# vbronetskyi/nclt-slam-project

Measured on AMD Instinct MI355X. Metric: relocalization frames/sec @640x480, 10k-landmark DB; Hamming-match HBM GB/s, higher is better.
Workload: dtype u8; 1 GPU; 640x480 BGR frames, 10000-record landmark DB (640000 descriptors, rows=fixed64), global relocalization tick per frame: ORB(500) + whole-DB mutual Hamming scan + top-25 PnP-RANSAC(200); frames resident in HBM, every frame's 96-byte result record written to pinned host memory by the tick's last kernel; distinct_frames=32, preroll_steps=20, streams=4, records=10000, descriptors=640000, parallelism=frames sharded across ranks, database replicated, no collective

## Files before the change

nclt-slam-project_amd/csrc/reloc_orb.hip:

```cpp
#include <math.h>

#include "../../include/reloc_orb_pattern.h"
#include "reloc_internal.h"
#include "reloc_pixels.h"

static_assert(HARRIS_CHUNK == 1024, "k_harris reads one dword per thread");

__constant__ signed char c_pattern[RELOC_ORB_NTESTS * 4];
__constant__ int c_umax[16] = {15, 15, 15, 15, 14, 14, 14, 13, 13, 12, 11, 10, 9, 8, 6, 3};
__constant__ signed char c_ring_dx[16] = {0, 1, 2, 3, 3, 3, 2, 1, 0, -1, -2, -3, -3, -3, -2, -1};
__constant__ signed char c_ring_dy[16] = {3, 3, 2, 1, 0, -1, -2, -3, -3, -3, -2, -1, 0, 1, 2, 3};

__device__ __forceinline__ int find_level(const int *base, int id)
{
    int l = 0;
#pragma unroll
    for (int k = 1; k < NLEV; ++k) l += id >= base[k];
    return l;
}


struct OrbBatch { OrbFrame f[RELOC_BATCH_MAX]; };

__device__ __forceinline__ void pyr_tab_index(const OrbTable *__restrict__ tab, const PyrTile &T, const int (&tbase)[NLEV + 1], int i,
                                              int &po, int &pc)
{
    int j = i, nw = 0, x0 = 0, y0 = 0, ox = 0, cx = 0, oy = 0, cy = 0;
#pragma unroll
    for (int k = 1; k < NLEV; ++k) {
        const bool m = i >= tbase[k];
        j = m ? i - tbase[k] : j;
        nw = m ? T.n[k][1] - T.n[k][0] : nw;
        x0 = m ? (int)T.n[k][0] : x0;
        y0 = m ? (int)T.n[k][2] : y0;
        ox = m ? tab->rz_off[k][0] : ox;
        cx = m ? tab->rz_off[k][1] : cx;
        oy = m ? tab->rz_off[k][2] : oy;
        cy = m ? tab->rz_off[k][3] : cy;
    }
    const bool isx = j < nw;
    const int p = isx ? x0 + j : y0 + j - nw;
    po = (isx ? ox : oy) + p;
    pc = (isx ? cx : cy) + p;
}

__device__ __forceinline__ int pyr_div(int q, float inv) { return (int)(((float)q + 0.5f) * inv); }

template <int CH, bool ALIGNED, int PYR_BS>
__device__ __forceinline__ void pyramid_body(const OrbTable *__restrict__ tab, const PyrTile *__restrict__ tiles,
                                                 const int32_t *__restrict__ rz, const uint8_t *__restrict__ src, int w, int h,
                                                 int sstride, int order_rgb, uint8_t *__restrict__ pyr, PyrLds lds,
                                                 int32_t *__restrict__ hist, int32_t *__restrict__ cand_cnt)
{
    extern __shared__ u32 s_pyr[];
    const int tid = threadIdx.x;
    if (blockIdx.x == 0) {
        for (int i = tid; i < NLEV * 256; i += PYR_BS) hist[i] = 0;
        if (tid < NLEV) cand_cnt[tid] = 0;
    }
    const PyrTile &T = tiles[blockIdx.x];
    uint8_t *const base = reinterpret_cast<uint8_t *>(s_pyr);
    u32 *const tabs = s_pyr + (lds.tabs >> 2);
    int tbase[NLEV + 1];
    tbase[1] = 0;
#pragma unroll
    for (int l = 1; l < NLEV; ++l) tbase[l + 1] = tbase[l] + (T.n[l][1] - T.n[l][0]) + (T.n[l][3] - T.n[l][2]);
    constexpr int TAB_IT = 1024 / PYR_BS, L0_IT = 1536 / PYR_BS;
    u32 tv[TAB_IT][2];
#pragma unroll
    for (int it = 0; it < TAB_IT; ++it) {
        const int i = tid + it * PYR_BS;
        tv[it][0] = tv[it][1] = 0;
        if (i < tbase[NLEV]) {
            int po, pc;
            pyr_tab_index(tab, T, tbase, i, po, pc);
            tv[it][0] = (u32)rz[po];
            tv[it][1] = (u32)rz[pc];
        }
    }
    const int x00 = T.n[0][0], y00 = T.n[0][2], qpr0 = (T.n[0][1] - x00 + 3) >> 2, nq0 = qpr0 * (T.n[0][3] - y00);
    const float inv0 = 1.0f / (float)(qpr0 > 0 ? qpr0 : 1);
    u32 fv[L0_IT][3];
#pragma unroll
    for (int it = 0; it < L0_IT; ++it) {
        const int q = tid + it * PYR_BS;
        if (q < nq0) {
            const int ry = pyr_div(q, inv0), x4 = x00 + (q - ry * qpr0) * 4;
            pyr_fetch<CH, ALIGNED>(src + (size_t)(y00 + ry) * sstride + CH * x4, x4, w, fv[it]);
        }
    }
#pragma unroll
    for (int it = 0; it < TAB_IT; ++it) {
        const int i = tid + it * PYR_BS;
        if (i < tbase[NLEV]) tabs[i] = tv[it][0] | tv[it][1] << 16;
    }
#pragma unroll
    for (int it = 0; it < L0_IT; ++it) {
        const int q = tid + it * PYR_BS;
        if (q < nq0) {
            const int ry = pyr_div(q, inv0), x4 = x00 + (q - ry * qpr0) * 4;
            reinterpret_cast<u32 *>(base + lds.lev[0])[q] = pyr_gray4<CH>(fv[it], x4, w, order_rgb);
        }
    }
    for (int q = tid + L0_IT * PYR_BS; q < nq0; q += PYR_BS) {
        const int ry = pyr_div(q, inv0), x4 = x00 + (q - ry * qpr0) * 4;
        u32 d[3];
        pyr_fetch<CH, ALIGNED>(src + (size_t)(y00 + ry) * sstride + CH * x4, x4, w, d);
        reinterpret_cast<u32 *>(base + lds.lev[0])[q] = pyr_gray4<CH>(d, x4, w, order_rgb);
    }
    for (int i = tid + TAB_IT * PYR_BS; i < tbase[NLEV]; i += PYR_BS) {
        int po, pc;
        pyr_tab_index(tab, T, tbase, i, po, pc);
        tabs[i] = (u32)rz[po] | (u32)rz[pc] << 16;
    }
    __syncthreads();
#pragma unroll
    for (int l = 0; l + 1 < NLEV; ++l) {
        const int sw = tab->lev[l].w, sh = tab->lev[l].h;
        const uint8_t *cur = base + lds.lev[l];
        u32 *nxt = reinterpret_cast<u32 *>(base + lds.lev[l + 1]);
        const int nx0 = T.n[l][0], ny0 = T.n[l][2], pitch = ((T.n[l][1] - nx0 + 3) >> 2) << 2;
        const int dx0 = T.n[l + 1][0], dx1 = T.n[l + 1][1], dh = T.n[l + 1][3] - T.n[l + 1][2];
        const int qpr = (dx1 - dx0 + 3) >> 2;
        const u32 *xt = tabs + tbase[l + 1], *yt = xt + (dx1 - dx0);
        const u32 one = 1u << RELOC_RESIZE_COEF_BITS;
        const float inv = 1.0f / (float)(qpr > 0 ? qpr : 1);
        for (int q = tid; q < qpr * dh; q += PYR_BS) {
            const int ry = pyr_div(q, inv), rx4 = (q - ry * qpr) * 4;
            const u32 ye = yt[ry];
            const int sy0 = (int)(ye & 0xFFFF), sy1 = sy0 + 1 < sh ? sy0 + 1 : sh - 1;
            const u32 b = ye >> 16;
            const uint8_t *r0 = cur + (sy0 - ny0) * pitch - nx0, *r1 = cur + (sy1 - ny0) * pitch - nx0;
            u32 out = 0;
#pragma unroll
            for (int k = 0; k < 4; ++k) {
                if (dx0 + rx4 + k < dx1) {
                    const u32 xe = xt[rx4 + k];
                    const int k0 = (int)(xe & 0xFFFF), k1 = k0 + 1 < sw ? k0 + 1 : sw - 1;
                    const u32 a = xe >> 16;
                    const u32 h0 = (u32)r0[k0] * (one - a) + (u32)r0[k1] * a;
                    const u32 h1 = (u32)r1[k0] * (one - a) + (u32)r1[k1] * a;
                    const u32 v = h0 * (one - b) + h1 * b;
                    out |= ((v + (1u << 15)) >> 16) << (8 * k);
                }
            }
            nxt[q] = out;
        }
        __syncthreads();
    }
#pragma unroll
    for (int l = 0; l < NLEV; ++l) {
        const OrbLevel L = tab->lev[l];
        const uint8_t *cur = base + lds.lev[l];
        const int nx0 = T.n[l][0], ny0 = T.n[l][2], pitch = ((T.n[l][1] - nx0 + 3) >> 2) << 2;
        const int x0 = T.o[l][0], x1 = T.o[l][1], y0 = T.o[l][2], oh = T.o[l][3] - y0;
        const int qpr = (x1 - x0) >> 2;
        uint8_t *dst = pyr + L.off;
        const float inv = 1.0f / (float)(qpr > 0 ? qpr : 1);
        for (int q = tid; q < qpr * oh; q += PYR_BS) {
            const int ry = pyr_div(q, inv), x4 = x0 + (q - ry * qpr) * 4;
            u32 v = 0;
            if (x4 < L.w) {
                v = *reinterpret_cast<const u32 *>(cur + (y0 + ry - ny0) * pitch + (x4 - nx0));
                if (x4 + 4 > L.w) v &= 0xFFFFFFFFu >> (8 * (x4 + 4 - L.w));
            }
            *reinterpret_cast<u32 *>(dst + (size_t)(y0 + ry) * L.stride + x4) = v;
        }
    }
}
template <int CH, bool ALIGNED, int PYR_BS>
__global__ __launch_bounds__(PYR_BS) void k_pyramid(const OrbTable *__restrict__ tab, const PyrTile *__restrict__ tiles,
                                                 const int32_t *__restrict__ rz, const uint8_t *__restrict__ src, int w, int h,
                                                 int sstride, int order_rgb, uint8_t *__restrict__ pyr, PyrLds lds,
                                                 int32_t *__restrict__ hist, int32_t *__restrict__ cand_cnt)
{
    RELOC_SMALL_KERNEL_PRIO();
    pyramid_body<CH, ALIGNED, PYR_BS>(tab, tiles, rz, src, w, h, sstride, order_rgb, pyr, lds, hist, cand_cnt);
}
template <int CH, bool ALIGNED, int PYR_BS>
__global__ __launch_bounds__(PYR_BS) void k_pyramid_batch(OrbBatch b, int w, int h, int sstride, int order_rgb, PyrLds lds)
{
    RELOC_SMALL_KERNEL_PRIO();
    const OrbFrame &F = b.f[blockIdx.y];
    pyramid_body<CH, ALIGNED, PYR_BS>(F.tab, F.tiles, F.rz, F.src, w, h, sstride, order_rgb, F.pyr, lds, F.hist, F.cand_cnt);
}

template <bool REFLECT>
__device__ __forceinline__ u32 halo_dword(const uint8_t *__restrict__ row, int gx, int w)
{
    if (gx >= 0 && gx + 4 <= w) return *reinterpret_cast<const u32 *>(row + gx);
    u32 v = 0;
#pragma unroll
    for (int k = 0; k < 4; ++k) {
        const int x = REFLECT ? reflect101(gx + k, w) : min(max(gx + k, 0), w - 1);
        v |= (u32)row[x] << (8 * k);
    }
    return v;
}

constexpr int BT_P = BT_W / 4 + 2;
static_assert(BT_W == 64 && BT_H == 16, "blur7_tile maps 256 lanes to 16 rows x 16 dwords");
__device__ __forceinline__ void blur7_tile(const OrbTable *__restrict__ tab, const uint8_t *__restrict__ pyr,
                                           uint8_t *__restrict__ blur, int bid)
{
    __shared__ u32 s_in[(BT_H + 6) * BT_P];
    __shared__ u32 s_h[(BT_H + 6) * BT_W / 2];
    const int l = find_level(tab->blur_tile_base, bid);
    const OrbLevel L = tab->lev[l];
    const int tile = bid - tab->blur_tile_base[l];
    const int tx = (L.w + BT_W - 1) / BT_W;
    const int x0 = (tile % tx) * BT_W, y0 = (tile / tx) * BT_H;
    const uint8_t *src = pyr + L.off;
    const int tid = threadIdx.x;
    const int r16 = tid >> 4, c16 = tid & 15;
    {
        const int e = tid - 6 * 16;
        const bool edge = e >= 0;
        const int rb = edge ? e >> 1 : BT_H + r16, db = edge ? (e & 1) * (BT_P - 1) : 1 + c16;
        const bool on = e < 2 * (BT_H + 6);
        const int gya = reflect101(y0 + r16 - 3, L.h), gyb = reflect101(y0 + rb - 3, L.h);
        const u32 va = halo_dword<true>(src + (size_t)gya * L.stride, x0 + 4 * c16, L.w);
        u32 vb = 0;
        if (on) vb = halo_dword<true>(src + (size_t)gyb * L.stride, x0 - 4 + 4 * db, L.w);
        s_in[r16 * BT_P + 1 + c16] = va;
        if (on) s_in[rb * BT_P + db] = vb;
    }
    __syncthreads();
    constexpr u32 W_LO = RELOC_BLUR_K0 | RELOC_BLUR_K1 << 8 | RELOC_BLUR_K2 << 16 | (u32)RELOC_BLUR_K3 << 24;
    constexpr u32 W_HI = RELOC_BLUR_K2 | RELOC_BLUR_K1 << 8 | RELOC_BLUR_K0 << 16;
    static_assert(RELOC_BLUR_K3 < 256 && 2 * (RELOC_BLUR_K0 + RELOC_BLUR_K1 + RELOC_BLUR_K2) + RELOC_BLUR_K3 <= 256, "blur taps");
#pragma unroll
    for (int t = 0; t < 2; ++t) {
        const int ry = t * BT_H + r16;
        if (ry < BT_H + 6) {
            const u32 *p = s_in + ry * BT_P + c16;
            const u32 d0 = p[0], d1 = p[1], d2 = p[2];
            u32 s[4];
#pragma unroll
            for (int k = 0; k < 4; ++k) {
                const u32 lo = k < 3 ? __builtin_amdgcn_alignbyte(d1, d0, 1 + k) : d1;
                const u32 hi = k < 3 ? __builtin_amdgcn_alignbyte(d2, d1, 1 + k) : d2;
                s[k] = __builtin_amdgcn_udot4(lo, W_LO, __builtin_amdgcn_udot4(hi, W_HI, 0u, false), false);
            }
            *reinterpret_cast<uint2 *>(s_h + ry * (BT_W / 2) + 2 * c16) = make_uint2(s[0] | s[1] << 16, s[2] | s[3] << 16);
        }
    }
    __syncthreads();
    {
        u32 c[7][4];
#pragma unroll
        for (int j = 0; j < 7; ++j) {
            const uint2 d = *reinterpret_cast<const uint2 *>(s_h + (r16 + j) * (BT_W / 2) + 2 * c16);
            c[j][0] = d.x & 0xFFFF; c[j][1] = d.x >> 16; c[j][2] = d.y & 0xFFFF; c[j][3] = d.y >> 16;
        }
        u32 out = 0;
#pragma unroll
        for (int k = 0; k < 4; ++k) {
            const u32 s = RELOC_BLUR_K0 * (c[0][k] + c[6][k]) + RELOC_BLUR_K1 * (c[1][k] + c[5][k]) +
                          RELOC_BLUR_K2 * (c[2][k] + c[4][k]) + RELOC_BLUR_K3 * c[3][k];
            out |= ((s + (1u << 15)) >> 16) << (8 * k);
        }
        const int gy = y0 + r16, gx = x0 + 4 * c16;
        if (gy < L.h && gx < L.stride) *reinterpret_cast<u32 *>(blur + L.off + (size_t)gy * L.stride + gx) = out;
    }
}

__device__ int fast_is_corner(const uint8_t *p, int stride, int thr)
{
    const int c = p[0];
    u32 bright = 0, dark = 0;
#pragma unroll
    for (int k = 0; k < 16; ++k) {
        const int v = (int)p[c_ring_dy[k] * stride + c_ring_dx[k]] - c;
        bright |= (u32)(v > thr) << k;
        dark |= (u32)(v < -thr) << k;
    }
    auto run9 = [](u32 m) {
        u32 x = m | (m << 16);
        u32 y = x & (x >> 1);
        y &= y >> 2;
        y &= y >> 4;
        y &= x >> 8;
        return (y & 0xFFFFu) != 0;
    };
    return run9(bright) ? 1 : (run9(dark) ? -1 : 0);
}

__device__ int fast_corner_score(const uint8_t *p, int stride, int thr, int sign)
{
    const int c = p[0];
    int v[16];
#pragma unroll
    for (int k = 0; k < 16; ++k) v[k] = sign * ((int)p[c_ring_dy[k] * stride + c_ring_dx[k]] - c);
    int m2[16], m4[16], best = 0;
#pragma unroll
    for (int k = 0; k < 16; ++k) m2[k] = min(v[k], v[(k + 1) & 15]);
#pragma unroll
    for (int k = 0; k < 16; ++k) m4[k] = min(m2[k], m2[(k + 2) & 15]);
#pragma unroll
    for (int k = 0; k < 16; ++k) {
        const int m8 = min(m4[k], m4[(k + 4) & 15]);
        const int m9 = min(m8, v[(k + 8) & 15]);
        best = max(best, m9);
    }
    return best > thr ? best - 1 : 0;
}

__device__ __forceinline__ bool fast_run9(u32 x)
{
    u32 y = x & (x >> 1);
    y &= y >> 2;
    y &= y >> 4;
    y &= x >> 8;
    return (y & 0xFFFFu) != 0;
}

struct FastQuad {
    u32 nb[2], nd[2];
    const u32 (*w)[3];
    __device__ __forceinline__ FastQuad(const u32 (&rows)[7][3], int thr) : w(rows)
    {
        const u32 c = rows[3][1];
        const u32 ce = c & 0x00FF00FFu, co = (c >> 8) & 0x00FF00FFu;
        const u32 t2 = (0x7FFFu - (u32)thr) * 0x00010001u;
        nb[0] = t2 - ce; nb[1] = t2 - co;
        nd[0] = t2 + ce; nd[1] = t2 + co;
    }
    template <int DX, int DY>
    __device__ __forceinline__ void flags(u32 (&tb)[2], u32 (&td)[2]) const
    {
        constexpr int b = 4 + DX, q = b >> 2, o = b & 3;
        constexpr u32 sel_e = (u32)o | 0x0C00u | (u32)(o + 2) << 16 | 0x0C000000u;
        constexpr u32 sel_o = (u32)(o + 1) | 0x0C00u | (u32)(o + 3) << 16 | 0x0C000000u;
        const u32 ve = __builtin_amdgcn_perm(w[DY + 3][q + 1], w[DY + 3][q], sel_e);
        const u32 vo = __builtin_amdgcn_perm(w[DY + 3][q + 1], w[DY + 3][q], sel_o);
        tb[0] = ve + nb[0]; tb[1] = vo + nb[1];
        td[0] = nd[0] - ve; td[1] = nd[1] - vo;
    }
    template <int K>
    __device__ __forceinline__ void ring(u32 (&tb)[2], u32 (&td)[2]) const
    {
        constexpr int dx[16] = {0, 1, 2, 3, 3, 3, 2, 1, 0, -1, -2, -3, -3, -3, -2, -1};
        constexpr int dy[16] = {3, 3, 2, 1, 0, -1, -2, -3, -3, -3, -2, -1, 0, 1, 2, 3};
        flags<dx[K], dy[K]>(tb, td);
    }
    __device__ __forceinline__ bool candidate() const
    {
        u32 b0[2], d0[2], b4[2], d4[2], b8[2], d8[2], b12[2], d12[2];
        ring<0>(b0, d0); ring<4>(b4, d4); ring<8>(b8, d8); ring<12>(b12, d12);
        u32 any = 0;
#pragma unroll
        for (int j = 0; j < 2; ++j) {
            any |= (b0[j] & b4[j]) | (b8[j] & b12[j]) | ((b0[j] | b4[j]) & (b8[j] | b12[j]));
            any |= (d0[j] & d4[j]) | (d8[j] & d12[j]) | ((d0[j] | d4[j]) & (d8[j] | d12[j]));
        }
        return (any & 0x80008000u) != 0;
    }
    template <int K>
    __device__ __forceinline__ void shift_in(u32 (&mb)[2], u32 (&md)[2]) const
    {
        u32 tb[2], td[2];
        ring<K>(tb, td);
#pragma unroll
        for (int j = 0; j < 2; ++j) {
            mb[j] = (tb[j] & 0x80008000u) | ((mb[j] >> 1) & 0x7FFF7FFFu);
            md[j] = (td[j] & 0x80008000u) | ((md[j] >> 1) & 0x7FFF7FFFu);
        }
        if constexpr (K < 15) shift_in<K + 1>(mb, md);
    }
    __device__ __forceinline__ void masks(u32 (&mb)[2], u32 (&md)[2]) const
    {
        mb[0] = mb[1] = md[0] = md[1] = 0;
        shift_in<0>(mb, md);
    }
};

constexpr int FT_P = FT / 4 + 3;
static_assert(FT == 32, "fast_nms_tile maps 256 lanes to 32 rows x 8 dwords");
template <bool MASKED, int THR>
__device__ __forceinline__ void fast_nms_tile(const OrbTable *__restrict__ tab, const uint8_t *__restrict__ pyr,
                                              uint8_t *__restrict__ nms, int32_t *__restrict__ hist, int bid,
                                              const uint8_t *__restrict__ mask)
{
    __shared__ u32 s_img4[(FT + 8) * FT_P];
    __shared__ u32 s_sc4[(FT + 2) * (FT + 4) / 4];
    __shared__ unsigned short s_corner[(FT + 2) * (FT + 2)];
    __shared__ int s_nc;
    __shared__ int s_hist[256];
    const uint8_t *const s_img = reinterpret_cast<const uint8_t *>(s_img4);
    uint8_t *const s_sc = reinterpret_cast<uint8_t *>(s_sc4);
    const int l = find_level(tab->fast_tile_base, bid);
    const OrbLevel L = tab->lev[l];
    const int tile = bid - tab->fast_tile_base[l];
    const int tx = L.stride / FT;
    const int x0 = (tile % tx) * FT, y0 = (tile / tx) * FT;
    const int tid = threadIdx.x;
    const int e = RELOC_ORB_EDGE;
    const int thr = THR ? THR : tab->fast_thr;
    uint8_t *out = nms + L.off;
    const bool live = L.quota > 0 && x0 + FT > e && x0 < L.w - e && y0 + FT > e && y0 < L.h - e;
    if (!live) {
        const int y = y0 + tid / 8, x = x0 + (tid % 8) * 4;
        if (y < L.h) *reinterpret_cast<u32 *>(out + (size_t)y * L.stride + x) = 0;
        return;
    }
    s_hist[tid] = 0;
    const uint8_t *src = pyr + L.off;
    const int IS = 4 * FT_P;
    {
        const int r16 = tid >> 4, c16 = tid & 15;
        u32 v[3];
#pragma unroll
        for (int t = 0; t < 3; ++t) {
            const int ry = 16 * t + r16;
            if (c16 < FT / 4 + 2 && ry < FT + 8) {
                const int gy = min(max(y0 + ry - 4, 0), L.h - 1);
                v[t] = halo_dword<false>(src + (size_t)gy * L.stride, x0 - 4 + 4 * c16, L.w);
            }
        }
#pragma unroll
        for (int t = 0; t < 3; ++t) {
            const int ry = 16 * t + r16;
            if (c16 < FT / 4 + 2 && ry < FT + 8) s_img4[ry * FT_P + c16] = v[t];
        }
    }
    for (int i = tid; i < (FT + 2) * (FT + 4) / 4; i += 256) s_sc4[i] = 0;
    if (tid == 0) s_nc = 0;
    __syncthreads();
    const int SS = FT + 4;
    {
        const int ry = 1 + (tid >> 3), g = tid & 7, rx = 1 + 4 * g;
        u32 w[7][3];
#pragma unroll
        for (int r = 0; r < 7; ++r)
#pragma unroll
            for (int q = 0; q < 3; ++q) w[r][q] = s_img4[(ry + r) * FT_P + g + q];
        const FastQuad Q(w, thr);
        if (__any(Q.candidate())) {
            u32 mb[2], md[2];
            Q.masks(mb, md);
            const int gy = y0 + ry - 1;
            const bool row_in = gy >= 3 && gy < L.h - 3;
#pragma unroll
            for (int k = 0; k < 4; ++k) {
                const u32 sel = (k & 2) ? 0x03020302u : 0x01000100u;
                const bool br = fast_run9(__builtin_amdgcn_perm(mb[k & 1], mb[k & 1], sel));
                const bool dk = fast_run9(__builtin_amdgcn_perm(md[k & 1], md[k & 1], sel));
                const int gx = x0 + rx - 1 + k;
                if ((br || dk) && row_in && gx >= 3 && gx < L.w - 3)
                    s_corner[atomicAdd(&s_nc, 1)] = (unsigned short)((ry << 6) | (rx + k) | (br ? 0 : 0x8000));
            }
        }
    }
    {
        const int i = tid;
        const int ry = i < FT + 2 ? 0 : (i < 2 * (FT + 2) ? FT + 1 : (i < 3 * FT + 4 ? i - (2 * FT + 3) : i - (3 * FT + 3)));
        const int rx = i < FT + 2 ? i : (i < 2 * (FT + 2) ? i - (FT + 2) : (i < 3 * FT + 4 ? 0 : FT + 1));
        const int gy = y0 + ry - 1, gx = x0 + rx - 1;
        int pol = 0;
        bool cand = false;
        const uint8_t *pc = s_img + (ry + 3) * IS + (rx + 3);
        const bool inside = i < 4 * FT + 4 && gx >= 3 && gx < L.w - 3 && gy >= 3 && gy < L.h - 3;
        if (inside) {
            const int c = pc[0];
            const int v0 = (int)pc[3 * IS] - c, v4 = (int)pc[3] - c, v8 = (int)pc[-3 * IS] - c, v12 = (int)pc[-3] - c;
            const int nb = (v0 > thr) + (v4 > thr) + (v8 > thr) + (v12 > thr);
            const int nd = (v0 < -thr) + (v4 < -thr) + (v8 < -thr) + (v12 < -thr);
            cand = nb >= 2 || nd >= 2;
        }
// ... 807 lines not shown
```

nclt-slam-project_amd/csrc/reloc_pixels.h:

```cpp
#pragma once
#include "reloc_internal.h"

typedef uint32_t u32;

__device__ __forceinline__ int reflect101(int p, int n)
{
    if (n == 1) return 0;
    while (p < 0 || p >= n) {
        if (p < 0) p = -p;
        if (p >= n) p = 2 * n - 2 - p;
    }
    return p;
}

__device__ __forceinline__ int gray_fixed(int b, int g, int r, int flags)
{
    const bool c15 = flags & RELOC_GRAY_FLAG_15BIT;
    const int cb = c15 ? RELOC_GRAY15_CB : RELOC_GRAY_CB, cg = c15 ? RELOC_GRAY15_CG : RELOC_GRAY_CG, cr = c15 ? RELOC_GRAY15_CR : RELOC_GRAY_CR;
    const int sh = c15 ? RELOC_GRAY15_SHIFT : RELOC_GRAY_SHIFT;
    return (b * cb + g * cg + r * cr + (1 << (sh - 1))) >> sh;
}
static inline int gray_flags(const reloc_ctx *ctx, int order)
{
    return (order & 1) | (ctx->prm.gray_coeff_bits == RELOC_GRAY15_SHIFT ? RELOC_GRAY_FLAG_15BIT : 0);
}

template <int CH, bool ALIGNED>
__device__ __forceinline__ void pyr_fetch(const uint8_t *sp, int x4, int w, u32 (&d)[3])
{
    if (ALIGNED) {
        const u32 *s4 = reinterpret_cast<const u32 *>(sp);
        d[0] = s4[0];
        if (CH == 3) { d[1] = s4[1]; d[2] = s4[2]; }
    } else {
        d[0] = d[1] = d[2] = 0;
#pragma unroll
        for (int k = 0; k < 4 * CH; ++k)
            if (x4 + k / CH < w) d[k >> 2] |= (u32)sp[k] << (8 * (k & 3));
    }
}

template <int CH>
__device__ __forceinline__ u32 pyr_gray4(const u32 (&d)[3], int x4, int w, int order_rgb)
{
    if (CH == 1) return d[0];
    u32 out = 0;
#pragma unroll
    for (int k = 0; k < 4; ++k) {
        int c[3];
#pragma unroll
        for (int j = 0; j < 3; ++j) { const int bi = 3 * k + j; c[j] = (d[bi >> 2] >> (8 * (bi & 3))) & 0xFF; }
        const int b = (order_rgb & 1) ? c[2] : c[0], r = (order_rgb & 1) ? c[0] : c[2];
        const int g = gray_fixed(b, c[1], r, order_rgb);
        if (x4 + k < w) out |= (u32)g << (8 * k);
    }
    return out;
}
```

Baseline: 7648 frames/s.

## Restructure pyramid kernel walks into column-major row strides with scalar tile loads

Replaces the per-element float division index decomposition in the pyramid build with a precomputed per-thread column/row walk, using a constant reciprocal table. Tile rectangles and the table are read through the constant address space so they load as scalars. The per-level resize hoists the x coefficients out of the row loop, packs output with a byte permute and masks the tail instead of branching. Gray conversion drops the per-pixel channel-swap select and the width check on aligned frames. These changes cut VALU and address arithmetic in a small ORB stage, at the cost of more intricate indexing and reliance on undocumented layout asserts.

```diff
diff --git a/nclt-slam-project_amd/csrc/reloc_orb.hip b/nclt-slam-project_amd/csrc/reloc_orb.hip
--- a/nclt-slam-project_amd/csrc/reloc_orb.hip
+++ b/nclt-slam-project_amd/csrc/reloc_orb.hip
@@ -22,29 +22,61 @@
 
 struct OrbBatch { OrbFrame f[RELOC_BATCH_MAX]; };
 
-__device__ __forceinline__ void pyr_tab_index(const OrbTable *__restrict__ tab, const PyrTile &T, const int (&tbase)[NLEV + 1], int i,
-                                              int &po, int &pc)
-{
-    int j = i, nw = 0, x0 = 0, y0 = 0, ox = 0, cx = 0, oy = 0, cy = 0;
-#pragma unroll
-    for (int k = 1; k < NLEV; ++k) {
-        const bool m = i >= tbase[k];
-        j = m ? i - tbase[k] : j;
-        nw = m ? T.n[k][1] - T.n[k][0] : nw;
-        x0 = m ? (int)T.n[k][0] : x0;
-        y0 = m ? (int)T.n[k][2] : y0;
-        ox = m ? tab->rz_off[k][0] : ox;
-        cx = m ? tab->rz_off[k][1] : cx;
-        oy = m ? tab->rz_off[k][2] : oy;
-        cy = m ? tab->rz_off[k][3] : cy;
-    }
+#define PYR_CONST __attribute__((address_space(4)))
+typedef const PYR_CONST OrbTable *PyrTabP;
+template <class P>
+__device__ __forceinline__ P pyr_reload(P p)
+{
+    asm volatile("" : "+s"(p));
+    return p;
+}
+struct PyrRect { int x0, x1, y0, y1; };
+__device__ __forceinline__ PyrRect pyr_rect(const PYR_CONST u32 *tile, int r)
+{
+    const u32 a = tile[2 * r], b = tile[2 * r + 1];
+    return {(int)(a & 0xFFFF), (int)(a >> 16), (int)(b & 0xFFFF), (int)(b >> 16)};
+}
+static_assert(offsetof(PyrTile, n) == 8 * NLEV && sizeof(PyrTile) == 16 * NLEV, "pyr_rect reads a rectangle as two dwords");
+
+__device__ __forceinline__ void pyr_tab_index(PyrTabP tab, const PyrRect &N, int l, int j, int &po, int &pc)
+{
+    const int nw = N.x1 - N.x0;
     const bool isx = j < nw;
-    const int p = isx ? x0 + j : y0 + j - nw;
-    po = (isx ? ox : oy) + p;
-    pc = (isx ? cx : cy) + p;
-}
-
-__device__ __forceinline__ int pyr_div(int q, float inv) { return (int)(((float)q + 0.5f) * inv); }
+    const int p = isx ? N.x0 + j : N.y0 + j - nw;
+    po = (isx ? tab->rz_off[l][0] : tab->rz_off[l][2]) + p;
+    pc = (isx ? tab->rz_off[l][1] : tab->rz_off[l][3]) + p;
+}
+
+__device__ __forceinline__ u32 pyr_byte(const uint8_t *p)
+{
+    return *(const volatile __attribute__((address_space(3))) uint8_t *)p;
+}
+
+constexpr int PYR_BS_MAX = 512;
+struct PyrInv { u32 v[PYR_BS_MAX + 1]; };
+constexpr PyrInv pyr_inv_table()
+{
+    PyrInv t{};
+    for (u32 d = 1; d <= PYR_BS_MAX; ++d) t.v[d] = ((1u << 22) + d - 1) / d;
+    return t;
+}
+__constant__ PyrInv c_pyr_inv = pyr_inv_table();
+
+struct PyrWalk { int cw, c, r, rstep; };
+template <int PYR_BS>
+__device__ __forceinline__ PyrWalk pyr_walk(int tid, int qpr)
+{
+    static_assert(PYR_BS <= PYR_BS_MAX, "c_pyr_inv");
+    PyrWalk W;
+    W.cw = qpr + (qpr == 0);
+    W.cw = W.cw < PYR_BS ? W.cw : PYR_BS;
+    const u32 m = c_pyr_inv.v[W.cw];
+    W.rstep = (int)((u32)PYR_BS * m >> 22);
+    const int r = (int)(__umul24(tid, m) >> 22);
+    W.c = tid - __mul24(r, W.cw);
+    W.r = r < W.rstep ? r : 1 << 20;
+    return W;
+}
 
 template <int CH, bool ALIGNED, int PYR_BS>
 __device__ __forceinline__ void pyramid_body(const OrbTable *__restrict__ tab, const PyrTile *__restrict__ tiles,
@@ -58,113 +90,137 @@
         for (int i = tid; i < NLEV * 256; i += PYR_BS) hist[i] = 0;
         if (tid < NLEV) cand_cnt[tid] = 0;
     }
-    const PyrTile &T = tiles[blockIdx.x];
+    const PYR_CONST u32 *const tile = (const PYR_CONST u32 *)(tiles + blockIdx.x);
+    const PyrTabP tabc = (PyrTabP)tab;
     uint8_t *const base = reinterpret_cast<uint8_t *>(s_pyr);
     u32 *const tabs = s_pyr + (lds.tabs >> 2);
-    int tbase[NLEV + 1];
+    int tbase[NLEV + 1], tmax = 0;
     tbase[1] = 0;
-#pragma unroll
-    for (int l = 1; l < NLEV; ++l) tbase[l + 1] = tbase[l] + (T.n[l][1] - T.n[l][0]) + (T.n[l][3] - T.n[l][2]);
-    constexpr int TAB_IT = 1024 / PYR_BS, L0_IT = 1536 / PYR_BS;
-    u32 tv[TAB_IT][2];
-#pragma unroll
-    for (int it = 0; it < TAB_IT; ++it) {
-        const int i = tid + it * PYR_BS;
-        tv[it][0] = tv[it][1] = 0;
-        if (i < tbase[NLEV]) {
+    u32 tv[NLEV][2];
+#pragma unroll
+    for (int l = 1; l < NLEV; ++l) {
+        const PyrRect N = pyr_rect(tile, NLEV + l);
+        tbase[l + 1] = tbase[l] + (N.x1 - N.x0) + (N.y1 - N.y0);
+        tmax = tmax > tbase[l + 1] - tbase[l] ? tmax : tbase[l + 1] - tbase[l];
+        tv[l][0] = tv[l][1] = 0;
+        if (tid < tbase[l + 1] - tbase[l]) {
             int po, pc;
-            pyr_tab_index(tab, T, tbase, i, po, pc);
-            tv[it][0] = (u32)rz[po];
-            tv[it][1] = (u32)rz[pc];
-        }
-    }
-    const int x00 = T.n[0][0], y00 = T.n[0][2], qpr0 = (T.n[0][1] - x00 + 3) >> 2, nq0 = qpr0 * (T.n[0][3] - y00);
-    const float inv0 = 1.0f / (float)(qpr0 > 0 ? qpr0 : 1);
+            pyr_tab_index(tabc, N, l, tid, po, pc);
+            tv[l][0] = (u32)rz[po];
+            tv[l][1] = (u32)rz[pc];
+        }
+    }
+    constexpr int L0_IT = 2048 / PYR_BS;
+    const PyrRect N0 = pyr_rect(tile, NLEV);
+    const int x00 = N0.x0, y00 = N0.y0, qpr0 = (N0.x1 - x00 + 3) >> 2, nh0 = N0.y1 - y00;
+    const PyrWalk W0 = pyr_walk<PYR_BS>(tid, qpr0);
+    u32 *const lev0 = reinterpret_cast<u32 *>(base + lds.lev[0]);
+    const bool col0 = W0.c < qpr0;
+    const int x40 = x00 + 4 * W0.c;
+    const uint8_t *const sp0 = src + (size_t)(y00 + W0.r) * sstride + CH * x40;
+    const size_t step0 = (size_t)W0.rstep * sstride;
     u32 fv[L0_IT][3];
 #pragma unroll
     for (int it = 0; it < L0_IT; ++it) {
-        const int q = tid + it * PYR_BS;
-        if (q < nq0) {
-            const int ry = pyr_div(q, inv0), x4 = x00 + (q - ry * qpr0) * 4;
-            pyr_fetch<CH, ALIGNED>(src + (size_t)(y00 + ry) * sstride + CH * x4, x4, w, fv[it]);
-        }
-    }
-#pragma unroll
-    for (int it = 0; it < TAB_IT; ++it) {
-        const int i = tid + it * PYR_BS;
-        if (i < tbase[NLEV]) tabs[i] = tv[it][0] | tv[it][1] << 16;
-    }
+        const int ry = W0.r + it * W0.rstep;
+        if (col0 && ry < nh0) pyr_fetch<CH, ALIGNED>(sp0 + it * step0, x40, w, fv[it]);
+    }
+#pragma unroll
+    for (int l = 1; l < NLEV; ++l)
+        if (tid < tbase[l + 1] - tbase[l]) tabs[tbase[l] + tid] = tv[l][0] | tv[l][1] << 16;
 #pragma unroll
     for (int it = 0; it < L0_IT; ++it) {
-        const int q = tid + it * PYR_BS;
-        if (q < nq0) {
-            const int ry = pyr_div(q, inv0), x4 = x00 + (q - ry * qpr0) * 4;
-            reinterpret_cast<u32 *>(base + lds.lev[0])[q] = pyr_gray4<CH>(fv[it], x4, w, order_rgb);
-        }
-    }
-    for (int q = tid + L0_IT * PYR_BS; q < nq0; q += PYR_BS) {
-        const int ry = pyr_div(q, inv0), x4 = x00 + (q - ry * qpr0) * 4;
-        u32 d[3];
-        pyr_fetch<CH, ALIGNED>(src + (size_t)(y00 + ry) * sstride + CH * x4, x4, w, d);
-        reinterpret_cast<u32 *>(base + lds.lev[0])[q] = pyr_gray4<CH>(d, x4, w, order_rgb);
-    }
-    for (int i = tid + TAB_IT * PYR_BS; i < tbase[NLEV]; i += PYR_BS) {
-        int po, pc;
-        pyr_tab_index(tab, T, tbase, i, po, pc);
-        tabs[i] = (u32)rz[po] | (u32)rz[pc] << 16;
+        const int ry = W0.r + it * W0.rstep;
+        if (col0 && ry < nh0) lev0[__mul24(ry, qpr0) + W0.c] = pyr_gray4<CH, ALIGNED>(fv[it], x40, w, order_rgb);
+    }
+    for (int c = W0.c; c < qpr0; c += W0.cw) {
+        const int x4 = x00 + 4 * c;
+        for (int ry = W0.r + (c == W0.c ? L0_IT * W0.rstep : 0); ry < nh0; ry += W0.rstep) {
+            u32 d[3];
+            pyr_fetch<CH, ALIGNED>(src + (size_t)(y00 + ry) * sstride + CH * x4, x4, w, d);
+            lev0[__mul24(ry, qpr0) + c] = pyr_gray4<CH, ALIGNED>(d, x4, w, order_rgb);
+        }
+    }
+    if (tmax > PYR_BS) {
+        int tb = 0;
+#pragma unroll 1
+        for (int l = 1; l < NLEV; ++l) {
+            const PyrRect N = pyr_rect(tile, NLEV + l);
+            const int n = (N.x1 - N.x0) + (N.y1 - N.y0);
+            for (int j = tid + PYR_BS; j < n; j += PYR_BS) {
+                int po, pc;
+                pyr_tab_index(tabc, N, l, j, po, pc);
+                tabs[tb + j] = (u32)rz[po] | (u32)rz[pc] << 16;
+            }
+            tb += n;
+        }
     }
     __syncthreads();
 #pragma unroll
     for (int l = 0; l + 1 < NLEV; ++l) {
-        const int sw = tab->lev[l].w, sh = tab->lev[l].h;
-        const uint8_t *cur = base + lds.lev[l];
         u32 *nxt = reinterpret_cast<u32 *>(base + lds.lev[l + 1]);
-        const int nx0 = T.n[l][0], ny0 = T.n[l][2], pitch = ((T.n[l][1] - nx0 + 3) >> 2) << 2;
-        const int dx0 = T.n[l + 1][0], dx1 = T.n[l + 1][1], dh = T.n[l + 1][3] - T.n[l + 1][2];
+        const PYR_CONST u32 *tl = pyr_reload(tile);
+        const PyrRect N = pyr_rect(tl, NLEV + l), D = pyr_rect(tl, NLEV + l + 1);
+        const int nx0 = N.x0, ny0 = N.y0, pitch = ((N.x1 - nx0 + 3) >> 2) << 2;
+        const int dx0 = D.x0, dx1 = D.x1, dh = D.y1 - D.y0;
         const int qpr = (dx1 - dx0 + 3) >> 2;
         const u32 *xt = tabs + tbase[l + 1], *yt = xt + (dx1 - dx0);
         const u32 one = 1u << RELOC_RESIZE_COEF_BITS;
-        const float inv = 1.0f / (float)(qpr > 0 ? qpr : 1);
-        for (int q = tid; q < qpr * dh; q += PYR_BS) {
-            const int ry = pyr_div(q, inv), rx4 = (q - ry * qpr) * 4;
-            const u32 ye = yt[ry];
-            const int sy0 = (int)(ye & 0xFFFF), sy1 = sy0 + 1 < sh ? sy0 + 1 : sh - 1;
-            const u32 b = ye >> 16;
-            const uint8_t *r0 = cur + (sy0 - ny0) * pitch - nx0, *r1 = cur + (sy1 - ny0) * pitch - nx0;
-            u32 out = 0;
+        const PyrWalk W = pyr_walk<PYR_BS>(tid, qpr);
+        const int org = lds.lev[l] - ny0 * pitch - nx0, nstep = W.rstep * qpr;
+        for (int c = W.c; c < qpr; c += W.cw) {
+            const int nv = dx1 - dx0 - 4 * c;
+            const u32 keep = nv >= 4 ? 0xFFFFFFFFu : ~(0xFFFFFFFFu << (8 * nv));
+            u32 k0[4], a[4], na[4];
 #pragma unroll
             for (int k = 0; k < 4; ++k) {
-                if (dx0 + rx4 + k < dx1) {
-                    const u32 xe = xt[rx4 + k];
-                    const int k0 = (int)(xe & 0xFFFF), k1 = k0 + 1 < sw ? k0 + 1 : sw - 1;
-                    const u32 a = xe >> 16;
-                    const u32 h0 = (u32)r0[k0] * (one - a) + (u32)r0[k1] * a;
-                    const u32 h1 = (u32)r1[k0] * (one - a) + (u32)r1[k1] * a;
-                    const u32 v = h0 * (one - b) + h1 * b;
-                    out |= ((v + (1u << 15)) >> 16) << (8 * k);
+                const u32 xe = xt[4 * c + (k < nv ? k : nv - 1)];
+                k0[k] = org + (xe & 0xFFFF);
+                a[k] = xe >> 16;
+                na[k] = one - a[k];
+            }
+            u32 *np = nxt + __mul24(W.r, qpr) + c;
+            for (int ry = W.r; ry < dh; ry += W.rstep, np += nstep) {
+                const u32 ye = yt[ry];
+                const u32 b = ye >> 16, nb = one - b;
+                const uint8_t *r0 = base + __umul24(ye & 0xFFFF, pitch), *r1 = r0 + pitch;
+                u32 v[4];
+#pragma unroll
+                for (int k = 0; k < 4; ++k) {
+                    const uint8_t *p0 = r0 + k0[k], *p1 = r1 + k0[k];
+                    const u32 h0 = (u32)p0[0] * na[k] + (u32)pyr_byte(p0 + 1) * a[k];
+                    const u32 h1 = (u32)p1[0] * na[k] + (u32)pyr_byte(p1 + 1) * a[k];
+                    u32 t = __umul24(h0, nb) + (1u << 15);
+                    asm("" : "+v"(t));
+                    v[k] = __umul24(h1, b) + t;
                 }
+                const u32 out = __builtin_amdgcn_perm(v[1], v[0], 0x0c0c0602u) | __builtin_amdgcn_perm(v[3], v[2], 0x06020c0cu);
+                *np = out & keep;
             }
-            nxt[q] = out;
         }
         __syncthreads();
     }
 #pragma unroll
     for (int l = 0; l < NLEV; ++l) {
-        const OrbLevel L = tab->lev[l];
+        const PyrTabP tabl = pyr_reload(tabc);
+        const PYR_CONST u32 *tl = pyr_reload(tile);
+        const int lw = tabl->lev[l].w, lstride = tabl->lev[l].stride;
         const uint8_t *cur = base + lds.lev[l];
-        const int nx0 = T.n[l][0], ny0 = T.n[l][2], pitch = ((T.n[l][1] - nx0 + 3) >> 2) << 2;
-        const int x0 = T.o[l][0], x1 = T.o[l][1], y0 = T.o[l][2], oh = T.o[l][3] - y0;
+        const PyrRect N = pyr_rect(tl, NLEV + l), O = pyr_rect(tl, l);
+        const int nx0 = N.x0, ny0 = N.y0, pitch = ((N.x1 - nx0 + 3) >> 2) << 2;
+        const int x0 = O.x0, x1 = O.x1, y0 = O.y0, oh = O.y1 - y0;
         const int qpr = (x1 - x0) >> 2;
-        uint8_t *dst = pyr + L.off;
-        const float inv = 1.0f / (float)(qpr > 0 ? qpr : 1);
-        for (int q = tid; q < qpr * oh; q += PYR_BS) {
-            const int ry = pyr_div(q, inv), x4 = x0 + (q - ry * qpr) * 4;
-            u32 v = 0;
-            if (x4 < L.w) {
-                v = *reinterpret_cast<const u32 *>(cur + (y0 + ry - ny0) * pitch + (x4 - nx0));
-                if (x4 + 4 > L.w) v &= 0xFFFFFFFFu >> (8 * (x4 + 4 - L.w));
-            }
-            *reinterpret_cast<u32 *>(dst + (size_t)(y0 + ry) * L.stride + x4) = v;
+        const PyrWalk W = pyr_walk<PYR_BS>(tid, qpr);
+        const int sstep = W.rstep * pitch;
+        const size_t dstep = (size_t)W.rstep * lstride;
+        for (int c = W.c; c < qpr; c += W.cw) {
+            const int x4 = x0 + 4 * c, nv = lw - x4;
+            const u32 keep = nv >= 4 ? 0xFFFFFFFFu : nv > 0 ? ~(0xFFFFFFFFu << (8 * nv)) : 0u;
+            const uint8_t *sp = nv > 0 ? cur + __mul24(y0 + W.r - ny0, pitch) + (x4 - nx0) : base;
+            const int sinc = nv > 0 ? sstep : 0;
+            uint8_t *dp = pyr + tabl->lev[l].off + (size_t)(y0 + W.r) * lstride + x4;
+            for (int ry = W.r; ry < oh; ry += W.rstep, sp += sinc, dp += dstep)
+                *reinterpret_cast<u32 *>(dp) = *reinterpret_cast<const u32 *>(sp) & keep;
         }
     }
 }
diff --git a/nclt-slam-project_amd/csrc/reloc_pixels.h b/nclt-slam-project_amd/csrc/reloc_pixels.h
--- a/nclt-slam-project_amd/csrc/reloc_pixels.h
+++ b/nclt-slam-project_amd/csrc/reloc_pixels.h
@@ -20,6 +20,13 @@
     const int sh = c15 ? RELOC_GRAY15_SHIFT : RELOC_GRAY_SHIFT;
     return (b * cb + g * cg + r * cr + (1 << (sh - 1))) >> sh;
 }
+__device__ __forceinline__ int gray_fixed_bytes(int c0, int c1, int c2, int flags)
+{
+    const bool c15 = flags & RELOC_GRAY_FLAG_15BIT, rgb = flags & 1;
+    const int cb = c15 ? RELOC_GRAY15_CB : RELOC_GRAY_CB, cg = c15 ? RELOC_GRAY15_CG : RELOC_GRAY_CG, cr = c15 ? RELOC_GRAY15_CR : RELOC_GRAY_CR;
+    const int sh = c15 ? RELOC_GRAY15_SHIFT : RELOC_GRAY_SHIFT;
+    return (c0 * (rgb ? cr : cb) + c1 * cg + c2 * (rgb ? cb : cr) + (1 << (sh - 1))) >> sh;
+}
 static inline int gray_flags(const reloc_ctx *ctx, int order)
 {
     return (order & 1) | (ctx->prm.gray_coeff_bits == RELOC_GRAY15_SHIFT ? RELOC_GRAY_FLAG_15BIT : 0);
@@ -40,7 +47,7 @@
     }
 }
 
-template <int CH>
+template <int CH, bool FULL = false>
 __device__ __forceinline__ u32 pyr_gray4(const u32 (&d)[3], int x4, int w, int order_rgb)
 {
     if (CH == 1) return d[0];
@@ -50,9 +57,8 @@
         int c[3];
 #pragma unroll
         for (int j = 0; j < 3; ++j) { const int bi = 3 * k + j; c[j] = (d[bi >> 2] >> (8 * (bi & 3))) & 0xFF; }
-        const int b = (order_rgb & 1) ? c[2] : c[0], r = (order_rgb & 1) ? c[0] : c[2];
-        const int g = gray_fixed(b, c[1], r, order_rgb);
-        if (x4 + k < w) out |= (u32)g << (8 * k);
+        const int g = gray_fixed_bytes(c[0], c[1], c[2], order_rgb);
+        if (FULL || x4 + k < w) out |= (u32)g << (8 * k);
     }
     return out;
 }
```

Measured after the change: 7694 frames/s (median of 6 runs). No clear change (+0.6%).
